# johnmatthewtennant/wab-gym

Measured on AMD Instinct MI355X. Metric: env-steps/sec (whole node) at batch=65536; obs bit-exact vs CPU ref, higher is better.
Workload: dtype u8

## Files before the change

wab_gym_amd/csrc/wab_build_guard.h:

```cpp
#pragma once

#if defined(WAB_STAMPS) || defined(WAB2_STAMPS) || defined(WAB_ROLL_FLOOR) || defined(WAB_WIDE_ROLL_FLOOR) || \
    defined(WAB2_ABLATE) || defined(WAB_ONLY_WAVE)
#if defined(WAB_PRODUCT_BUILD)
#error "a diagnostic macro (WAB_STAMPS, WAB2_STAMPS, WAB_ROLL_FLOOR, WAB_WIDE_ROLL_FLOOR, WAB2_ABLATE, WAB_ONLY_WAVE) is set in the product build"
#elif !defined(WAB_DIAGNOSTIC_BUILD)
#error "diagnostic macros need -DWAB_DIAGNOSTIC_BUILD and an output outside the product library (tools/build_variants.sh)"
#endif
#endif

#ifndef WAB_RULES_INSTANCE
#define WAB_RULES_INSTANCE 1
#endif
#ifndef WAB_ROLL_HOIST
#define WAB_ROLL_HOIST 1
#endif
#if defined(WAB_PRODUCT_BUILD) && (WAB_RULES_INSTANCE != 1 || WAB_ROLL_HOIST != 1)
#error "WAB_RULES_INSTANCE / WAB_ROLL_HOIST are A/B switches: the product build takes their defaults"
#endif

#if defined(WAB_DIAGNOSTIC_BUILD) && !defined(__HIP_DEVICE_COMPILE__)
extern "C" __attribute__((weak, visibility("default"))) int wab_diagnostic_build(void) { return 1; }
#endif
```

wab_gym_amd/csrc/wab_step_small.hip:

```cpp
#include <hip/hip_runtime.h>

#include "wab_default_rules.h"
#include "wab_feat.h"
#include "wab_policy_dev.h"

#ifndef WAB_ROLL_THROTTLE
#define WAB_ROLL_THROTTLE 0
#endif
#ifndef WAB_ROLL_OBS_NT
#define WAB_ROLL_OBS_NT 1
#endif
namespace wab {

#ifdef WAB_STAMPS
#define SMALL_STAMP(slot)                                                                \
  do {                                                                                   \
    if (lane == 0 && p.stamps && (!ROLL || t == p.n_steps / 2))                          \
      p.stamps[(size_t)blockIdx.x * kStampStride + (slot)] = __builtin_amdgcn_s_memrealtime();      \
  } while (0)
#else
#define SMALL_STAMP(slot) do {} while (0)
#endif

namespace {
// ... 249 lines not shown
constexpr int kW1ResetPrio = 2;

template <bool ROLL>
__device__ __forceinline__ void role_prio(uint32_t level, int t, bool rot) {
  if (ROLL && rot)
    set_prio_dyn((level >= 2u ? 1u : 0u) + 2u * (((blockIdx.x >> 8) + (uint32_t)t) & 1u));
  else
    set_prio_dyn(level);
}
constexpr int kStripW1 = 8;
__device__ __forceinline__ M128 strip_of(const Params& p, const Lds& s, int lane, int dir) {
  return strip_cells(p, dir, s.strip[lane] | s.strip[64 + lane]);
}

__device__ __forceinline__ void scan_log(const Params& p, const Head& h, const uint32_t* lxy, const uint32_t* lrem,
                                         int i0, int ne, int& found, int& found_rem, M128& gone) {
#pragma unroll
  for (int k = 0; k < 4; ++k) {
    const bool in = i0 + k < ne;
    const uint32_t v = lxy[k];
    const int r = (int)lrem[k];
    if (in && v == h.cpos) {
      found = i0 + k;
      found_rem = r;
    }
    const int ddx = h.ox - xy_x(v), ddy = h.oy - xy_y(v);
    set_bit_if(gone, (uint32_t)((ddx + p.cw) * p.H + ddy + p.ch), in && r == 0 && abs(ddx) <= p.cw && abs(ddy) <= p.ch);
  }
}

__device__ __forceinline__ void stream_set_ostrich(const Params& p, uint32_t* stream, uint32_t ebit, int role) {
  const uint32_t ccb = (uint32_t)(p.cw * p.H + p.ch);
  if (p.restrict_view && m_test(view_mask_of(p, role), ccb)) return;
  const uint32_t bit = ebit + 2u * (uint32_t)p.WH + ccb;
  atomicOr(&stream[bit >> 5], 1u << (bit & 31u));
}

__device__ __forceinline__ void render_s(const Params& p, const Lds& s, int lane, uint32_t info, int dir) {
  const uint32_t WH = (uint32_t)p.WH;
  const uint32_t ebit = (uint32_t)lane * (uint32_t)p.OB;
  const int role = (int)((info >> 8) & 0xFFu);
  M128 wp = m_unpack(s.wolfp[lane]);
  M128 bp = m_or(m_unpack(s.bushp[lane]), m_andn(strip_of(p, s, lane, dir), m_unpack(s.gone[lane])));
  if (p.restrict_view) {
    const M128 vm = view_mask_of(p, role);
    wp = m_andn(wp, vm);
    bp = m_andn(bp, vm);
  }
  if (wp.lo | wp.hi) stream_or128(s.stream, ebit, wp);
  stream_or128(s.stream, ebit + WH, bp);
  stream_set_ostrich(p, s.stream, ebit, role);
}


#ifndef WAB_STORE_WHOLE
#define WAB_STORE_WHOLE 1
#endif
constexpr uint32_t kUnits11 = 64u * 363u / 16u;
template <int NT, int K0, int K1, int I0>
__device__ __forceinline__ void store_units_whole11(uint8_t* out, uint32_t* stream, int lane) {
  typedef uint32_t u32x4 __attribute__((ext_vector_type(4)));
  typedef u32x4 __attribute__((may_alias)) u32x4_any;
  static_assert(I0 % 64 == 0 && NT % 64 == 0, "a wave's units of one k are contiguous");
  static_assert((uint32_t)(I0 + NT * K0) < kUnits11, "the wave has a unit");
  const uint16_t* s16 = reinterpret_cast<const uint16_t*>(stream) + I0;
  uint32_t v[K1 - K0];
  uint32_t share_end = 0u;
#pragma unroll
  for (int k = K0; k < K1; ++k) {
    const uint32_t u0 = (uint32_t)(I0 + NT * k);
    if (u0 + 63u < kUnits11) v[k - K0] = (uint32_t)s16[lane + NT * k];
    else if (u0 < kUnits11) v[k - K0] = (uint32_t)s16[min((uint32_t)lane, kUnits11 - 1u - u0) + NT * k];
    else v[k - K0] = 0u;
    if (u0 < kUnits11) share_end = min((u0 + 64u) * 2u, (kUnits11 * 2u + 15u) & ~15u);
  }
#pragma unroll
  for (int i = 0; i < (K1 - K0 + 7) / 8; ++i) {
    const uint32_t k = (uint32_t)(K0 + 8 * i) + ((uint32_t)lane >> 3);
    const uint32_t byte = ((uint32_t)I0 + (uint32_t)NT * k) * 2u + 16u * ((uint32_t)lane & 7u);
    *reinterpret_cast<u32x4_any*>(reinterpret_cast<uint8_t*>(stream) + min(byte, share_end - 16u)) = u32x4{0u, 0u, 0u, 0u};
  }
  if (!out) return;
  typedef uint8_t __attribute__((address_space(1))) g_u8;
  typedef u32x4 __attribute__((address_space(1))) g_u32x4;
  g_u8* base = (g_u8*)out;
  uint32_t base_off = 0u;
#pragma unroll
  for (int k = K0; k < K1; ++k) {
    const uint32_t u0 = (uint32_t)(I0 + NT * k);
    if (u0 >= kUnits11) continue;
    const uint32_t adv = ((uint32_t)(NT * k) * 16u - base_off) & ~4095u;
    if (adv) {
      base += adv;
      base_off += adv;
      asm("" : "+s"(base));
    }
    if (u0 + 63u >= kUnits11 && u0 + (uint32_t)lane >= kUnits11) continue;
    u32x4 q;
#pragma unroll
    for (int b = 0; b < 4; ++b) q[b] = (((v[k - K0] >> (4 * b)) & 0xFu) * 0x00204081u) & 0x01010101u;
    g_u32x4* dst = (g_u32x4*)base + (uint32_t)(I0 + lane + NT * k - (int)(base_off / 16u));
    if (WAB_ROLL_OBS_NT) __builtin_nontemporal_store(q, dst);
    else *dst = q;
  }
}

template <int G, int NT, int NK, int I0>
__device__ __forceinline__ void store_units_nt(const Params& p, uint8_t* planes, uint32_t* stream, int lane) {
  const int64_t g0 = (int64_t)blockIdx.x * 64;
  const uint32_t OB = (uint32_t)p.OB;
  if (WAB_STORE_WHOLE && G == 11 && p.B - g0 >= 64) {
    store_units_whole11<NT, 0, NK, I0>(planes ? planes + (size_t)g0 * OB : nullptr, stream, lane);
    return;
  }
  const int idx = I0 + lane;
  const uint32_t full = ((uint32_t)min((int64_t)64, p.B - g0) * OB) >> 4;
  uint8_t* out = planes + (size_t)g0 * OB;
  uint16_t* s16 = reinterpret_cast<uint16_t*>(stream);
  uint32_t v[NK];
#pragma unroll
  for (int k = 0; k < NK; ++k) {
    const uint32_t u = (uint32_t)(idx + NT * k);
    v[k] = u < full ? (uint32_t)s16[u] : 0u;
  }
#pragma unroll
  for (int k = 0; k < NK; ++k) {
    const uint32_t u = (uint32_t)(idx + NT * k);
    if (u < full) s16[u] = 0;
  }
  if (!planes) return;
#pragma unroll
  for (int k = 0; k < NK; ++k) {
    const uint32_t u = (uint32_t)(idx + NT * k);
    if (u >= full) continue;
    typedef uint32_t u32x4 __attribute__((ext_vector_type(4)));
    u32x4 q;
#pragma unroll
    for (int b = 0; b < 4; ++b) q[b] = (((v[k] >> (4 * b)) & 0xFu) * 0x00204081u) & 0x01010101u;
    if (WAB_ROLL_OBS_NT) __builtin_nontemporal_store(q, reinterpret_cast<u32x4*>(out) + u);
    else reinterpret_cast<u32x4*>(out)[u] = q;
  }
}

#ifndef WAB_ROLL_FLOOR
#define WAB_ROLL_FLOOR 0
#endif

struct CarryHdr {
  uint4 hdr;
};
struct CarryW0 {
  uint8_t* prev_planes;
  uint32_t* prev_stream;
  uint4 hdr;
  double food;
  uint32_t bw[4];
  uint32_t lxy[4], lrem[4];
};
template <int SLOTS>
struct CarryW2 {
  static constexpr int NR = carry_reg_slots(SLOTS);
  uint8_t* prev_planes;
  uint32_t* prev_stream;
  uint4 hdr;
  uint32_t wr[NR > 0 ? NR : 1];
  uint32_t live;
};

template <typename C>
struct CarryPtr {
  uint8_t* prev_planes;
  uint32_t* prev_stream;
  C c;
};

__device__ __forceinline__ int act_of(const Lds& s, int lane) {
  return (int)reinterpret_cast<const int8_t*>(s.act)[lane];
}

__device__ __forceinline__ void prefetch_actions(const Params& p, const Lds& s, int lane) {
  const int64_t g0 = (int64_t)blockIdx.x * 64;
  const int8_t* a = p.actions + p.B + g0;
  if (g0 + 64 <= p.B && (reinterpret_cast<uintptr_t>(a) & 3u) == 0u) {
    typedef const uint32_t __attribute__((address_space(4))) CU32;
    CU32* c = (CU32*)reinterpret_cast<uintptr_t>(a);
    asm volatile("" : "+s"(c));
    uint32_t v[16];
#pragma unroll
    for (int k = 0; k < 16; ++k) v[k] = c[k];
    uint32_t d = 0;
#pragma unroll
    for (int k = 0; k < 16; ++k) d = lane == k ? v[k] : d;
    if (lane < 16) s.act[lane] = d;
  } else {
    const int8_t v = g0 + lane < p.B ? a[lane] : (int8_t)0;
    reinterpret_cast<int8_t*>(s.act)[lane] = v;
  }
}

// ... 132 lines not shown
    bw0 = carry->bw[0];
    bw1 = carry->bw[1];
    bw2 = carry->bw[2];
    bw3 = carry->bw[3];
#pragma unroll
    for (int i = 0; i < 4; ++i) {
      lxy[i] = carry->lxy[i];
      lrem[i] = carry->lrem[i];
    }
  } else {
  hr = head_fetch<COLD>(p, g, active);
  {
    const int64_t gl = active ? g : 0;
    food = cold_of<COLD>(p).food[gl];
    bw0 = cold_of<COLD>(p).bushmap[gl];
    if (p.WHW > 1) bw1 = cold_of<COLD>(p).bushmap[p.B + gl];
    if (p.WHW > 2) bw2 = cold_of<COLD>(p).bushmap[2 * p.B + gl];
    if (p.WHW > 3) bw3 = cold_of<COLD>(p).bushmap[3 * p.B + gl];
#pragma unroll
    for (int i = 0; i < 4; ++i) {
      const int64_t at = (int64_t)min(i, p.eaten_cap - 1) * p.B + gl;
      lxy[i] = cold_of<COLD>(p).eaten_xy[at];
      lrem[i] = cold_of<COLD>(p).eaten_rem[at];
    }
  }
  opaque_head(hr);
  opaque(food);
  opaque(bw0);
  opaque(bw1);
  opaque(bw2);
  opaque(bw3);
#pragma unroll
  for (int i = 0; i < 4; ++i) {
    opaque(lxy[i]);
    opaque(lrem[i]);
  }
  }
  if (!active) {
    food = 0.0;
    bw0 = bw1 = bw2 = bw3 = 0u;
  }
  const bool init = !ROLL || t == 0;
  if (init) {
    uint4* z = reinterpret_cast<uint4*>(s.stream);
    for (uint32_t i = lane; i < L.stream_words / 4u; i += 64) z[i] = make_uint4(0u, 0u, 0u, 0u);
  }
  if (ROLL && pol) hr.a = act_of(s, lane);
  const Head h = head_decode(p, g, active, hr);
  if (lane == 0 && init) {
    s.flag[0] = 0u;
    s.flag[1] = 0u;
  }
  if (init) lds_barrier();
  int ne = (int)misc_ne(h.hdr.z), ndep = (int)misc_ndep(h.hdr.z);
  if (ROLL && t == 0) {
    for (int i = 4; i < kSmallLog; ++i)
      if (active && i < ne && i < p.eaten_cap) {
        s.elxy[(i - 4) * 64 + lane] = cold_of<COLD>(p).eaten_xy[(int64_t)i * p.B + g];
        s.elrem[(i - 4) * 64 + lane] = cold_of<COLD>(p).eaten_rem[(int64_t)i * p.B + g];
      }
    __builtin_amdgcn_s_waitcnt(0);
  }
  const int status_old = (int)misc_status(h.hdr.z);
  const int role = h.role;
  M128 bm = m_make(bw0, bw1, bw2, bw3);
  if (h.dir == DIR_RIGHT || h.dir == DIR_UP) shl128(bm.lo, bm.hi, h.dir == DIR_RIGHT ? p.H : 1);
  else if (h.dir == DIR_LEFT || h.dir == DIR_DOWN) shr128(bm.lo, bm.hi, h.dir == DIR_LEFT ? p.H : 1);
  {
    const M128 valid = m_make(sreg(p.small_masks[2][0]), sreg(p.small_masks[2][1]), sreg(p.small_masks[2][2]),
                              sreg(p.small_masks[2][3]));
    const M128 col0 = m_make(sreg(p.small_masks[0][0]), sreg(p.small_masks[0][1]), sreg(p.small_masks[0][2]),
                             sreg(p.small_masks[0][3]));
    const M128 coll = m_make(sreg(p.small_masks[1][0]), sreg(p.small_masks[1][1]), sreg(p.small_masks[1][2]),
                             sreg(p.small_masks[1][3]));
    const bool up = h.dir == DIR_UP, down = h.dir == DIR_DOWN;
    const M128 drop = {sel64(up, col0.lo, 0ull) | sel64(down, coll.lo, 0ull),
                       sel64(up, col0.hi, 0ull) | sel64(down, coll.hi, 0ull)};
    bm = m_andn(m_and(bm, valid), drop);
  }
  SMALL_STAMP(1);
  SMALL_STAMP(2);
  int found = -1, found_rem = 0;
  M128 gone = {0ull, 0ull};
  scan_log(p, h, lxy, lrem, 0, ne, found, found_rem, gone);
  bm = m_andn(bm, gone);
  bool center_bush = m_test(bm, ccb);
  if (ne > 4 && (center_bush || (ndep > 0 && h.dir != DIR_STAY))) {
    const int i_hbm = ROLL ? kSmallLog : 4;
    if (ROLL)
      for (int i0 = 4; i0 < ne && i0 < kSmallLog; i0 += 4) {
        uint32_t exy[4], erem[4];
#pragma unroll
        for (int k = 0; k < 4; ++k) {
          exy[k] = s.elxy[(i0 + k - 4) * 64 + lane];
          erem[k] = s.elrem[(i0 + k - 4) * 64 + lane];
        }
        scan_log(p, h, exy, erem, i0, ne, found, found_rem, gone);
      }
    for (int i0 = i_hbm; i0 < ne; i0 += 4) {
      uint32_t exy[4] = {0u, 0u, 0u, 0u}, erem[4] = {0u, 0u, 0u, 0u};
#pragma unroll
      for (int k = 0; k < 4; ++k)
        if (i0 + k < ne) {
          exy[k] = cold_of<COLD>(p).eaten_xy[(int64_t)(i0 + k) * p.B + g];
          erem[k] = cold_of<COLD>(p).eaten_rem[(int64_t)(i0 + k) * p.B + g];
        }
      scan_log(p, h, exy, erem, i0, ne, found, found_rem, gone);
    }
    bm = m_andn(bm, gone);
    center_bush = m_test(bm, ccb);
  }
  SMALL_STAMP(7);
  s.bushp[lane] = m_pack(bm);
  s.gone[lane] = m_pack(gone);
  int rem = found_rem;
  if (found < 0) {
    rem = 0;
    if (center_bush) {
      lds_await(p, s.flag);
      rem = (int)s.cval[lane];
    }
  }
  SMALL_STAMP(8);
  double reward = 0.0;
  unsigned long long eaten_of = 0;
  const bool ate = rem > 0 && status_old == 0 && (role == 1 || p.lookout_only);
  if (ate) {
    food = food + p.fill;
    food = food < 0.0 ? 0.0 : (food > 1.0 ? 1.0 : food);
    reward += p.r_eat;
    bool logged = true;
    if (ROLL && found >= 0 && found < 4) {
#pragma unroll
      for (int k = 0; k < 4; ++k)
        if (found == k) lrem[k] = (uint32_t)(rem - 1);
    } else if (ROLL && found < 0 && ne < 4 && ne < p.eaten_cap) {
#pragma unroll
      for (int k = 0; k < 4; ++k)
        if (ne == k) {
          lxy[k] = h.cpos;
          lrem[k] = (uint32_t)(rem - 1);
        }
      ne += 1;
    } else if (ROLL && found >= 4 && found < kSmallLog) {
      s.elrem[(found - 4) * 64 + lane] = (uint8_t)(rem - 1);
    } else if (ROLL && found < 0 && ne >= 4 && ne < kSmallLog && ne < p.eaten_cap) {
      s.elxy[(ne - 4) * 64 + lane] = h.cpos;
      s.elrem[(ne - 4) * 64 + lane] = (uint8_t)(rem - 1);
      ne += 1;
    } else if (found >= 0) {
      cold_of<COLD>(p).eaten_rem[(int64_t)found * p.B + g] = (uint8_t)(rem - 1);
    } else if (ne < p.eaten_cap) {
      cold_of<COLD>(p).eaten_xy[(int64_t)ne * p.B + g] = h.cpos;
      cold_of<COLD>(p).eaten_rem[(int64_t)ne * p.B + g] = (uint8_t)(rem - 1);
      ne += 1;
    } else {
      eaten_of += 1;
      logged = false;
    }
    if (rem == 1) {
      m_clear(bm, ccb);
      if (logged) ndep += 1;
    }
  }
  food = food - p.hunger;
  const bool starved = food <= 0.0;
  if (starved) food = 0.0;
  s.info[lane] = (starved ? 1u : 0u) | ((uint32_t)role << 8) | ((uint32_t)ne << 16) | ((uint32_t)ndep << 24);
  SMALL_STAMP(3);
  lds_barrier();
  role_prio<ROLL>(1, t, p.features != nullptr);

  const bool killed = s.kill[lane] != 0u;
  const int status = starved ? 1 : killed ? 2 : status_old;
  const bool done = env_done(p, h, starved, killed);
  {
    const double r_finish = sreg(p.r_finish), r_turn = sreg(p.r_turn);
    const double r_starve = sreg(p.r_starve), r_killed = sreg(p.r_killed);
    reward += sel_f64(status == 0, sel_f64(done, r_finish, r_turn), sel_f64(status == 1, r_starve, r_killed));
  }
  const bool job = active && done && p.autoreset;
  if (ROLL && p.returns)
    s.rcode[64 * t + lane] = reward_code(ate, status, done);
  if (active) {
    const int ft = (int)ceil(food * (double)p.turns_empty);
    __builtin_nontemporal_store((float)reward, p.reward + g);
    __builtin_nontemporal_store((uint8_t)(done ? 1 : 0), p.done + g);
    uint8_t* fts = reinterpret_cast<uint8_t*>(sel64(job, (uint64_t)p.t_food_turns, (uint64_t)p.food_turns));
    uint8_t* rls = reinterpret_cast<uint8_t*>(sel64(job, (uint64_t)p.t_role, (uint64_t)p.role));
    uint8_t* sts = reinterpret_cast<uint8_t*>(sel64(job, (uint64_t)p.t_status, (uint64_t)p.status));
    if (!job || (!ROLL && p.t_planes)) {
      fts[g] = (uint8_t)ft;
      rls[g] = (uint8_t)role;
      sts[g] = (uint8_t)status;
    }
    if (p.features && !job) s.scal[lane] = (uint32_t)ft | ((uint32_t)role << 8) | ((uint32_t)status << 16);
    if (!job) {
      bm = m_or(bm, m_andn(strip_of(p, s, lane, h.dir), gone));
      if (!ROLL || last) {
        cold_of<COLD>(p).bushmap[g] = m_word<0>(bm);
        if (p.WHW > 1) cold_of<COLD>(p).bushmap[p.B + g] = m_word<1>(bm);
        if (p.WHW > 2) cold_of<COLD>(p).bushmap[2 * p.B + g] = m_word<2>(bm);
        if (p.WHW > 3) cold_of<COLD>(p).bushmap[3 * p.B + g] = m_word<3>(bm);
        cold_of<COLD>(p).food[g] = food;
      }
    }
  }
  if (eaten_of) atomicAdd(&cold_of<COLD>(p).counters[CTR_EATEN_OVERFLOW], eaten_of);
  if (active && !h.valid_action) atomicAdd(&cold_of<COLD>(p).counters[CTR_BAD_ACTIONS], 1ull);
  if (blockIdx.x == 0 && threadIdx.x == 0)
    atomicAdd(&cold_of<COLD>(p).counters[CTR_STEPS], (unsigned long long)p.B);
  const unsigned long long jm = __ballot(job);
  if (lane == 0 && jm) atomicAdd(&p.block_resets[blockIdx.x], (unsigned long long)__popcll(jm));
  if (ROLL && carry->prev_stream) store_units_nt<G, 128, 12, 0>(p, carry->prev_planes, carry->prev_stream, lane);
  SMALL_STAMP(4);
  lds_barrier();
  if (!ROLL && p.t_planes) {
    unsigned long long wolf_of = 0;
    if (jm) {
      uint8_t* tout = p.t_planes + (size_t)g0 * OB;
      for (unsigned long long jj = jm; jj; jj &= jj - 1) {
        const uint32_t ee = (uint32_t)(__ffsll(jj) - 1);
        for (uint32_t k = lane; k < OB; k += 64) {
          const uint32_t bit = ee * OB + k;
          tout[bit] = (uint8_t)((s.stream[bit >> 5] >> (bit & 31)) & 1u);
        }
      }
      asm volatile("s_waitcnt lgkmcnt(0)" ::: "memory");
      if (job) {
        const uint32_t ebit = (uint32_t)lane * OB;
        stream_clear(s.stream, ebit, OB);
        const int j = __popcll(jm & ((1ull << lane) - 1ull));
        const uint2 kq = *reinterpret_cast<const uint2*>(&s.jkey[2 * j]);
        const int role2 = new_episode_a<SLOTS>(p, s, h, g, kq.x, kq.y, ebit, wolf_of);
        new_episode_b(p, s, g, j, ebit, role2);
      }
    }
    if (wolf_of) atomicAdd(&cold_of<COLD>(p).counters[CTR_WOLF_OVERFLOW], wolf_of);
    lds_barrier();
  }
  if constexpr (ROLL) {
    if (!last) {
      if (job) {
        const NewEp n = carry_of(s, lane);
        const int j = __popcll(jm & ((1ull << lane) - 1ull));
        const uint4 nb = *reinterpret_cast<const uint4*>(&s.jbm[4 * j]);
        carry->hdr = new_header(n, h);
        carry->food = n.food;
        carry->bw[0] = nb.x;
        carry->bw[1] = nb.y;
        carry->bw[2] = nb.z;
// ... 12 lines not shown
        carry->lxy[i] = lxy[i];
        carry->lrem[i] = lrem[i];
      }
    } else if (active && !job) {
#pragma unroll
      for (int i = 0; i < 4; ++i)
        if (i < ne && i < p.eaten_cap) {
          cold_of<COLD>(p).eaten_xy[(int64_t)i * p.B + g] = lxy[i];
          cold_of<COLD>(p).eaten_rem[(int64_t)i * p.B + g] = (uint8_t)lrem[i];
        }
      for (int i = 4; i < kSmallLog; ++i)
        if (i < ne && i < p.eaten_cap) {
          cold_of<COLD>(p).eaten_xy[(int64_t)i * p.B + g] = s.elxy[(i - 4) * 64 + lane];
          cold_of<COLD>(p).eaten_rem[(int64_t)i * p.B + g] = s.elrem[(i - 4) * 64 + lane];
        }
    }
  }
  if (ROLL && last && p.returns) rollout_returns<COLD>(p, s, g, active, lane);
  SMALL_STAMP(5);
  return jm;
}

template <int G, bool ROLL = false, bool COLD = false>
__device__ __forceinline__ unsigned long long draws_wave(const Params& p, const SmallLayout& L, uint32_t* lds, int lane,
                                                         CarryHdr* carry = nullptr, int t = 0, bool last = true,
                                                         bool pol = false) {
  const Lds s = lds_of(lds, L);
  const int64_t g = (int64_t)blockIdx.x * 64 + lane;
  SMALL_STAMP(10);
  role_prio<ROLL>(2, t, p.features != nullptr);
  HeadRaw hr;
  if (ROLL && t > 0) {
    hr.hdr = carry->hdr;
    hr.a = act_of(s, lane);
  } else {
  hr = head_fetch<COLD>(p, g, g < p.B);
  {
    const int nthr = p.max_berries;
    uint64_t tv[4];
#pragma unroll
    for (int k = 0; k < 4; ++k) tv[k] = cold_of<COLD>(p).thresholds[min(64 * k + lane, max(nthr, 1) - 1)];
    opaque_head(hr);
#pragma unroll
    for (int k = 0; k < 4; ++k) opaque(tv[k]);
#pragma unroll
    for (int k = 0; k < 4; ++k)
      if (64 * k + lane < nthr) s.thr[64 * k + lane] = tv[k];
    if (lane == 0) bush_thr_pads(s.thr, nthr);
  }
  }
  if (ROLL && pol) hr.a = act_of(s, lane);
  const Head h = head_decode(p, g, g < p.B, hr);
  if (!ROLL || t == 0) lds_barrier();
  SMALL_STAMP(30);
  const uint64_t ek = mix64(h.kenv ^ (uint64_t)h.hdr.w);
  const uint32_t b0 = (uint32_t)ek, b1 = (uint32_t)(ek >> 32);
  SMALL_STAMP(31);
  s.cval[lane] =
      (uint32_t)bush_value_fast(s.thr, p.max_berries, draw_U(h.cpos, make_ts(SITE_BUSH, 0, 0), b0, b1), p.bush_power);
  lds_publish(s.flag);
  role_prio<ROLL>(0, t, p.features != nullptr);
  if (p.features && !p.restrict_view && !ROLL)
    early_view_zeros(p, 0u, (uint32_t)min((int64_t)32, p.B - (int64_t)blockIdx.x * 64), lane);
  SMALL_STAMP(11);
  s.strip[lane] = strip_draws(p, h, b0, b1, 0, kStripW1);
  SMALL_STAMP(12);
  lds_barrier();
  const uint32_t info = s.info[lane];
  const bool killed = s.kill[lane] != 0u;
  const bool job = h.active && p.autoreset && env_done(p, h, info_starved(info), killed);
  const unsigned long long jm = __ballot(job);
  if (jm) {
    if (ROLL) role_prio<ROLL>(kW1ResetPrio, t, p.features != nullptr);
    if (job) {
      const uint64_t ek2 = mix64(h.kenv ^ (uint64_t)(h.hdr.w + 1u));
      const int j = __popcll(jm & ((1ull << lane) - 1ull));
      *reinterpret_cast<uint2*>(&s.jkey[2 * j]) = make_uint2((uint32_t)ek2, (uint32_t)(ek2 >> 32));
    }
    reset_chunk(p, s.tiles, s.jkey, __popcll(jm), 0u, lane, s.jbm);
    lds_publish(&s.flag[1]);
    if (ROLL) role_prio<ROLL>(0, t, p.features != nullptr);
  }
  if (h.active && (!job || (!ROLL && p.t_planes))) {
    render_s(p, s, lane, info, h.dir);
  }
  if (ROLL && !last && !pol) prefetch_actions(p, s, lane);
  SMALL_STAMP(13);
  lds_barrier();
  if (!ROLL && p.t_planes) lds_barrier();
  SMALL_STAMP(14);
  if (ROLL && lane == 0) {
    s.flag[0] = 0u;
    s.flag[1] = 0u;
  }
  if (ROLL && !last) {
    const uint32_t status = info_starved(info) ? 1u : killed ? 2u : misc_status(h.hdr.z);
    carry->hdr = job ? new_header(carry_of(s, lane), h)
                     : make_uint4(h.cpos, (uint32_t)h.turn, misc_pack((uint32_t)h.role, status, 0u, 0u, 0u), h.hdr.w);
  }
  return jm;
}

template <int SLOTS, int G, bool ROLL = false, bool COLD = false>
__device__ __forceinline__ unsigned long long wolves_wave(const Params& p, const SmallLayout& L, uint32_t* lds, int lane,
                                                          CarryW2<SLOTS>* carry = nullptr, int t = 0, bool last = true,
                                                          bool pol = false) {
  const Lds s = lds_of(lds, L);
  const int64_t g = (int64_t)blockIdx.x * 64 + lane;
  const bool active = g < p.B;
  SMALL_STAMP(16);
#ifndef WAB_SPEC_WOLVES
#define WAB_SPEC_WOLVES 8
#endif
  constexpr int kSpecSlots = SLOTS < WAB_SPEC_WOLVES ? SLOTS : WAB_SPEC_WOLVES;
  uint32_t wr[SLOTS];
#pragma unroll
  for (int k = 0; k < SLOTS; ++k) wr[k] = 0u;
  HeadRaw hr;
  const bool carried = ROLL && t > 0;
  if (carried) {
    hr.hdr = carry->hdr;
    hr.a = act_of(s, lane);
    constexpr int NR = CarryW2<SLOTS>::NR;
#pragma unroll
    for (int k = 0; k < SLOTS; ++k) wr[k] = k < NR ? carry->wr[k < NR ? k : 0] : s.wcar[(k - NR) * 64 + lane];
  } else {
  {
    const int64_t gl = active ? g : 0;
#pragma unroll
    for (int k = 0; k < kSpecSlots; ++k) wr[k] = cold_of<COLD>(p).wolves[(int64_t)k * p.B + gl];
  }
  hr = head_fetch<COLD>(p, g, active);
  opaque_head(hr);
#pragma unroll
  for (int k = 0; k < kSpecSlots; ++k) opaque(wr[k]);
  }
  if (ROLL && pol) hr.a = act_of(s, lane);
  const Head h = head_decode(p, g, active, hr);
  if (!ROLL || t == 0) lds_barrier();
  SMALL_STAMP(28);
  const int nw = (int)misc_nw(h.hdr.z);
  if (!carried) {
#pragma unroll
    for (int k = kSpecSlots; k < SLOTS; ++k)
      if (k < nw) wr[k] = cold_of<COLD>(p).wolves[(int64_t)k * p.B + g];
  }
  const uint64_t ek = mix64(h.kenv ^ (uint64_t)h.hdr.w);
  const uint32_t b0 = (uint32_t)ek, b1 = (uint32_t)(ek >> 32);
  uint32_t live = carried ? (h.active ? carry->live : 0u) : nw >= 32 ? ~0u : ((1u << nw) - 1u);

  {
    uint32_t keep = 0;
#pragma unroll
    for (int g4 = 0; g4 < SLOTS; g4 += 4) {
      const uint32_t live4 = (live >> g4) & 0xFu;
      if (!live4) continue;
      uint32_t h1[4], hh[4], ts[4];
#pragma unroll
      for (int q = 0; q < 4; ++q) {
        const int k = g4 + q;
        uint32_t occ = 0;
#pragma unroll
        for (int t = 0; t < k; ++t) occ += (((live >> t) & 1u) && wr[t] == wr[k]) ? 1u : 0u;
        ts[q] = make_ts(SITE_DESPAWN, occ, h.turn);
        h1[q] = wr[k] ^ b0;
      }
      fmix32x4(h1);
#pragma unroll
      for (int q = 0; q < 4; ++q) hh[q] = h1[q] ^ ts[q] ^ b1;
      fmix32x4(hh);
      uint32_t kp = 0, tie = 0;
#pragma unroll
      for (int q = 0; q < 4; ++q) {
        kp |= (hh[q] > p.keep_th ? 1u : 0u) << q;
        tie |= (hh[q] == p.keep_th ? 1u : 0u) << q;
      }
      if (tie & live4) {
#pragma unroll
        for (int q = 0; q < 4; ++q)
          if (((tie >> q) & 1u) && draw_lo21(h1[q], ts[q], b0) >= p.keep_tl) kp |= 1u << q;
      }
      keep |= (kp & live4) << g4;
    }
    live = keep;
  }
  SMALL_STAMP(29);
  M128 wolfp = {0ull, 0ull};
  bool kill = false;
#pragma unroll
  for (int g4 = 0; g4 < SLOTS; g4 += 4) {
    if (!((live >> g4) & 0xFu)) continue;
#pragma unroll
    for (int q = 0; q < 4; ++q) {
      const int k = g4 + q;
      const bool on = (live >> k) & 1u;
      int wx = xy_x(wr[k]), wy = xy_y(wr[k]);
      if (p.wolves_can_move) {
        const int ddx = h.ox - wx, ddy = h.oy - wy;
        const bool alongx = abs(ddx) >= abs(ddy);
        wx += alongx ? sgn(ddx) : 0;
        wy += alongx ? 0 : sgn(ddy);
        wr[k] = xy_pack(wx, wy);
      }
      const int ddx = h.ox - wx, ddy = h.oy - wy;
      set_bit_if(wolfp, (uint32_t)((ddx + p.cw) * p.H + ddy + p.ch), on && abs(ddx) <= p.cw && abs(ddy) <= p.ch);
      kill |= on && ddx == 0 && ddy == 0;
    }
  }
  kill = kill && !p.god_mode;
  s.wolfp[lane] = m_pack(wolfp);
  s.kill[lane] = kill ? 1u : 0u;
  SMALL_STAMP(17);
  SMALL_STAMP(18);
  lds_barrier();
  const uint32_t info = s.info[lane];
  const bool starved = info_starved(info);
  const bool job = active && p.autoreset && env_done(p, h, starved, kill);

  unsigned long long wolf_of = 0;
  const M128 spawn = m_unpack(s.spawn[lane]);
  if (active && (spawn.lo | spawn.hi)) {
#pragma unroll
    for (int half = 0; half < 2; ++half) {
      uint64_t bits = half ? spawn.hi : spawn.lo;
      while (bits) {
        const int b = __ffsll((unsigned long long)bits) - 1;
        bits &= bits - 1;
        const int r = 64 * half + b;
        const uint32_t w = xy_add(h.cpos, G == 11 ? ring11(r) : cold_of<COLD>(p).tables[p.ring_at + r]);
        bool placed = false;
#pragma unroll
        for (int k = 0; k < SLOTS; ++k)
          if (!placed && !((live >> k) & 1u)) { wr[k] = w; live |= 1u << k; placed = true; }
        if (!placed) wolf_of += 1;
      }
    }
  }
  if (active && !job && (!ROLL || last)) {
    int n = 0;
#pragma unroll
    for (int k = 0; k < SLOTS; ++k)
      if ((live >> k) & 1u) cold_of<COLD>(p).wolves[(int64_t)(n++) * p.B + g] = wr[k];
    const uint32_t status = starved ? 1u : kill ? 2u : misc_status(h.hdr.z);
    cold_of<COLD>(p).hdr[g] = make_uint4(h.cpos, (uint32_t)h.turn,
                          misc_pack((info >> 8) & 0xFFu, status, (uint32_t)n, (info >> 16) & 0xFFu, info >> 24),
                          h.hdr.w);
  }
  if (wolf_of) atomicAdd(&cold_of<COLD>(p).counters[CTR_WOLF_OVERFLOW], wolf_of);
  const unsigned long long jm = __ballot(job);
  if (ROLL && carry->prev_stream) store_units_nt<G, 128, 12, 64>(p, carry->prev_planes, carry->prev_stream, lane);
  SMALL_STAMP(19);
  lds_barrier();
  if (!ROLL && p.t_planes) lds_barrier();
  SMALL_STAMP(20);
  if (ROLL && !last) {
    if (job) {
      const NewEp n = carry_of(s, lane);
      M128 m = n.wolves;
      constexpr int NR = CarryW2<SLOTS>::NR;
#pragma unroll
      for (int k = 0; k < SLOTS; ++k) {
        const bool any = (m.lo | m.hi) != 0ull;
        const uint32_t c = m.lo ? (uint32_t)(__ffsll((unsigned long long)m.lo) - 1)
                                : (uint32_t)(__ffsll((unsigned long long)m.hi) + 63);
        const uint32_t w = any ? s.tiles[any ? c : 0u] : 0u;
        if (k < NR) carry->wr[k < NR ? k : 0] = w;
        else s.wcar[(k - NR) * 64 + lane] = w;
        if (any) m_clear(m, c);
      }
      carry->live = n.nw >= 32u ? ~0u : ((1u << n.nw) - 1u);
// ... 13 lines not shown
                              h.hdr.w);
    }
  }
  return jm;
}

template <int SLOTS, int G, bool ROLL = false, bool COLD = false>
__device__ __forceinline__ unsigned long long ring_wave(const Params& p, const SmallLayout& L, uint32_t* lds, int lane,
                                                        CarryHdr* carry = nullptr, int t = 0, bool last = true,
                                                        bool pol = false) {
  const Lds s = lds_of(lds, L);
  const int64_t g = (int64_t)blockIdx.x * 64 + lane;
  SMALL_STAMP(22);
  if (ROLL) role_prio<ROLL>(0, t, p.features != nullptr);
  HeadRaw hr;
  if (ROLL && t > 0) {
    hr.hdr = carry->hdr;
    hr.a = act_of(s, lane);
    reinterpret_cast<uint4*>(s.jbm)[lane] = make_uint4(0u, 0u, 0u, 0u);
  } else {
  hr = head_fetch<COLD>(p, g, g < p.B);
  if constexpr (G == 11) {
    for (int c = lane; c < 121; c += 64) s.tiles[c] = xy_pack(5 - c / 11, 5 - c % 11);
  } else {
    uint32_t tv[2];
#pragma unroll
    for (int k = 0; k < 2; ++k) tv[k] = cold_of<COLD>(p).tables[min(64 * k + lane, p.WH - 1)];
#pragma unroll
    for (int k = 0; k < 2; ++k)
      if (64 * k + lane < p.WH) s.tiles[64 * k + lane] = tv[k];
  }
  reinterpret_cast<uint4*>(s.jbm)[lane] = make_uint4(0u, 0u, 0u, 0u);
  {
    const int n = p.n_gap + 1;
    uint64_t gv[3];
#pragma unroll
    for (int k = 0; k < 3; ++k) gv[k] = cold_of<COLD>(p).gap[min(64 * k + lane, n - 1)];
    opaque_head(hr);
#pragma unroll
    for (int k = 0; k < 3; ++k) opaque(gv[k]);
#pragma unroll
    for (int k = 0; k < 3; ++k)
      if (64 * k + lane < n) s.gap[64 * k + lane] = gv[k];
  }
  }
  if (p.features) {
    uint4* z = reinterpret_cast<uint4*>(lds + L.fbits);
    const uint32_t nz = ROLL && t > 0 ? L.ftab - L.fbits : L.fzero;
    for (uint32_t i = lane; i < nz / 4u; i += 64) z[i] = make_uint4(0u, 0u, 0u, 0u);
  }
  if (ROLL && pol) hr.a = act_of(s, lane);
  const Head h = head_decode(p, g, g < p.B, hr);
  if (!ROLL || t == 0) lds_barrier();
  if (p.features) {
    if (!ROLL || t == 0)
      feat_tables_build(feat_tables_at(lds + L.ftab, p.W / 2 + p.H / 2 + 1), p.W, p.H, p.W / 2 + p.H / 2 + 1, lane, 64);
    if (!p.restrict_view && !ROLL)
      early_view_zeros(p, 32u, (uint32_t)max((int64_t)0, min((int64_t)32, p.B - (int64_t)blockIdx.x * 64 - 32)), lane);
  }
  const uint64_t ek = mix64(h.kenv ^ (uint64_t)h.hdr.w);
  const uint32_t b0 = (uint32_t)ek, b1 = (uint32_t)(ek >> 32);
  M128 spawn = {0ull, 0ull};
  if (p.wolves_on && h.active)
    spawn_hits(s.gap, p.R, p.gap_full_th, p.gap_full_tl, p.gap_ring_th, p.gap_ring_tl, p.gap_inv_l2, h.turn, b0, b1, [&](int r) { m_set(spawn, (uint32_t)r); });
  s.spawn[lane] = m_pack(spawn);
  s.strip[64 + lane] = strip_draws(p, h, b0, b1, kStripW1, 1 << 30);
  SMALL_STAMP(23);
  lds_barrier();
  role_prio<ROLL>(3, t, p.features != nullptr);
  const bool job = h.active && p.autoreset && env_done(p, h, info_starved(s.info[lane]), s.kill[lane] != 0u);
  const unsigned long long jm = __ballot(job);
  int role2 = 0;
  if (jm) {
    const int j = __popcll(jm & ((1ull << lane) - 1ull));
    uint32_t* jkey = s.jkey + 2 * 64;
    uint64_t ek2 = 0;
    if (job) {
      ek2 = mix64(h.kenv ^ (uint64_t)(h.hdr.w + 1u));
      *reinterpret_cast<uint2*>(&jkey[2 * j]) = make_uint2((uint32_t)ek2, (uint32_t)(ek2 >> 32));
    }
    const int n_jobs = __popcll(jm);
    for (uint32_t c0 = 64; c0 < (uint32_t)p.WH; c0 += 64)
      reset_chunk(p, s.tiles, jkey, n_jobs, c0, lane, s.jbm);
    SMALL_STAMP(24);
    if (ROLL || !p.t_planes) {
      unsigned long long wolf_of = 0;
      const uint32_t ebit = (uint32_t)lane * (uint32_t)p.OB;
      if (job) role2 = new_episode_a<SLOTS, ROLL, COLD>(p, s, h, g, (uint32_t)ek2, (uint32_t)(ek2 >> 32), ebit, wolf_of, last);
      lds_await(p, &s.flag[1]);
      SMALL_STAMP(9);
      if (job) new_episode_b<COLD>(p, s, g, j, ebit, role2, !ROLL || last);
      if (wolf_of) atomicAdd(&cold_of<COLD>(p).counters[CTR_WOLF_OVERFLOW], wolf_of);
    }
  }
  SMALL_STAMP(25);
  lds_barrier();
  if (!ROLL && p.t_planes) lds_barrier();
  SMALL_STAMP(26);
  if (ROLL && !last) {
    const uint32_t status = info_starved(s.info[lane]) ? 1u : s.kill[lane] != 0u ? 2u : misc_status(h.hdr.z);
    carry->hdr = job ? new_header(carry_of(s, lane), h)
                     : make_uint4(h.cpos, (uint32_t)h.turn, misc_pack((uint32_t)h.role, status, 0u, 0u, 0u), h.hdr.w);
  }
  return jm;
}

template <int G, int K0, int K1, int WAVE>
__device__ __forceinline__ void store_units_of(const Params& p, uint32_t* stream, int lane) {
  const int64_t g0 = (int64_t)blockIdx.x * 64;
  const uint32_t OB = (uint32_t)p.OB;
  if (WAB_STORE_WHOLE && G == 11 && p.B - g0 >= 64) {
    store_units_whole11<256, K0, K1, 64 * WAVE>(p.planes + (size_t)g0 * OB, stream, lane);
    return;
  }
  const int tid = 64 * WAVE + lane;
  const uint32_t full = ((uint32_t)min((int64_t)64, p.B - g0) * OB) >> 4;
  uint8_t* out = p.planes + (size_t)g0 * OB;
  uint16_t* s16 = reinterpret_cast<uint16_t*>(stream);
  uint32_t v[K1 - K0];
#pragma unroll
  for (int k = K0; k < K1; ++k) {
    const uint32_t u = (uint32_t)tid + 256u * (uint32_t)k;
    v[k - K0] = u < full ? (uint32_t)s16[u] : 0u;
  }
#pragma unroll
  for (int k = K0; k < K1; ++k) {
    const uint32_t u = (uint32_t)tid + 256u * (uint32_t)k;
    if (u < full) s16[u] = 0;
  }
#pragma unroll
  for (int k = K0; k < K1; ++k) {
    const uint32_t u = (uint32_t)tid + 256u * (uint32_t)k;
    if (u >= full) break;
    typedef uint32_t u32x4 __attribute__((ext_vector_type(4)));
    u32x4 q;
#pragma unroll
    for (int b = 0; b < 4; ++b) q[b] = (((v[k - K0] >> (4 * b)) & 0xFu) * 0x00204081u) & 0x01010101u;
    if (WAB_ROLL_OBS_NT) __builtin_nontemporal_store(q, reinterpret_cast<u32x4*>(out) + u);
    else reinterpret_cast<u32x4*>(out)[u] = q;
  }
}

template <bool CLEAR = false>
__device__ __forceinline__ void store_obs(const Params& p, uint32_t* stream, int tid) {
  const int64_t g0 = (int64_t)blockIdx.x * 64;
  const uint32_t OB = (uint32_t)p.OB;
  const uint32_t limit = (uint32_t)min((int64_t)64, p.B - g0) * OB;
  uint8_t* out = p.planes + (size_t)g0 * OB;
  const uint16_t* s16 = reinterpret_cast<const uint16_t*>(stream);
  const uint32_t full = limit >> 4;
  uint32_t v[6];
#pragma unroll
  for (int k = 0; k < 6; ++k) {
    const uint32_t u = (uint32_t)tid + 256u * (uint32_t)k;
    v[k] = u < full ? (uint32_t)s16[u] : 0u;
  }
  if constexpr (CLEAR) {
    uint16_t* w16 = reinterpret_cast<uint16_t*>(stream);
#pragma unroll
    for (int k = 0; k < 6; ++k) {
      const uint32_t u = (uint32_t)tid + 256u * (uint32_t)k;
      if (u < full) w16[u] = 0;
    }
  }
#pragma unroll
  for (int k = 0; k < 6; ++k) {
    const uint32_t u = (uint32_t)tid + 256u * (uint32_t)k;
    if (u >= full) break;
    typedef uint32_t u32x4 __attribute__((ext_vector_type(4)));
    u32x4 q;
#pragma unroll
    for (int b = 0; b < 4; ++b) q[b] = (((v[k] >> (4 * b)) & 0xFu) * 0x00204081u) & 0x01010101u;
#ifndef WAB_STEP_OBS_NT
#define WAB_STEP_OBS_NT 1
#endif
    if (WAB_STEP_OBS_NT) __builtin_nontemporal_store(q, reinterpret_cast<u32x4*>(out) + u);
    else reinterpret_cast<u32x4*>(out)[u] = q;
  }
  for (uint32_t b = (full << 4) + tid; b < limit; b += 256)
    out[b] = (uint8_t)((stream[b >> 5] >> (b & 31)) & 1u);
#ifdef WAB_STAMPS
  asm volatile("s_waitcnt vmcnt(0)" ::: "memory");
  if ((tid & 63) == 0 && p.stamps) {
    const int slot[4] = {6, 15, 21, 27};
    p.stamps[(size_t)blockIdx.x * kStampStride + slot[tid >> 6]] = __builtin_amdgcn_s_memrealtime();
  }
#endif
}

template <bool ROLL = false, bool POLICY = false>
__device__ __forceinline__ void step_features(const Params& p, const SmallLayout& L, uint32_t* lds, int wave,
                                              int lane, int t = 0, float* rows = nullptr) {
  const int md = p.W / 2 + p.H / 2 + 1;
  const uint32_t F = (uint32_t)pragmatic_dim(md, p.turns_empty), WH = (uint32_t)p.WH;
  const int64_t g0 = (int64_t)blockIdx.x * 64;
  const uint32_t n_active = (uint32_t)min((int64_t)64, p.B - g0);
  const uint32_t* stream = lds + L.stream;
  uint32_t* ob = lds + L.fbits;
  if (ROLL && (uint32_t)lane < n_active) {
    const uint32_t ebit = (uint32_t)lane * (uint32_t)p.OB, at = (uint32_t)lane * F;
    const FeatTables ft = feat_tables_at(lds + L.ftab, md);
    if (wave <= 1) {
      uint32_t near, second;
      plane_nearest(ft, md, stream_get128(stream, ebit + (uint32_t)wave * WH, WH), near, second);
      emit_nearest(ob, at, wave, md, near, second);
    } else if (wave == 2) {
#pragma unroll
      for (int pl = 0; pl < 2; ++pl) {
        int counts[4];
        plane_counts(ft, stream_get128(stream, ebit + (uint32_t)pl * WH, WH), counts);
        emit_counts(ob, at, pl, md, counts);
      }
    } else {
      const uint32_t sc = lds[L.scal + lane];
      const uint32_t role = (sc >> 8) & 0xFFu;
      const uint32_t sb_bit = ebit + WH + (uint32_t)(md / 2) * (uint32_t)p.S + (uint32_t)(md / 2);
      emit_scalars(ob, at, md, p.turns_empty, (stream[sb_bit >> 5] >> (sb_bit & 31u)) & 1u, sc & 0xFFu, role,
                   sc >> 16, p.restrict_view != 0, view_mask_of(p, (int)role));
    }
  } else if ((uint32_t)lane < n_active && wave < 3) {
    const uint32_t ebit = (uint32_t)lane * (uint32_t)p.OB, at = (uint32_t)lane * F;
    if (wave <= 1) {
      uint32_t near, second;
      int counts[4];
      plane_features(feat_tables_at(lds + L.ftab, md), md, stream_get128(stream, ebit + (uint32_t)wave * WH, WH), near,
                     second, counts);
      emit_plane(ob, at, wave, md, near, second, counts);
    } else {
      const uint32_t sc = lds[L.scal + lane];
      const uint32_t role = (sc >> 8) & 0xFFu;
      const uint32_t sb_bit = ebit + WH + (uint32_t)(md / 2) * (uint32_t)p.S + (uint32_t)(md / 2);
      emit_scalars(ob, at, md, p.turns_empty, (stream[sb_bit >> 5] >> (sb_bit & 31u)) & 1u, sc & 0xFFu, role,
                   sc >> 16, p.restrict_view != 0, view_mask_of(p, (int)role));
    }
  }
#ifdef WAB_STAMPS
  const auto stamp = [&](int slot) {
    if (ROLL && threadIdx.x == 0 && p.stamps && t == p.n_steps / 2)
      p.stamps[(size_t)blockIdx.x * kStampStride + slot] = __builtin_amdgcn_s_memrealtime();
  };
// ... 187 lines not shown
  p.block_resets = r.block_resets; p.n_steps = r.n_steps;
  p.t_planes = nullptr; p.t_food_turns = r.food_turns; p.t_role = r.role; p.t_status = r.status;
}

template <int SLOTS, int G, bool FEAT, bool ROLL, bool RULES, bool POLICY>
__global__ __launch_bounds__(256) __attribute__((amdgpu_waves_per_eu(POLICY ? 2 : ROLL ? 4 : 1))) void wab_step_small(Params p0) {
  static_assert(!POLICY || (FEAT && ROLL), "the policy build is a build of wab_rollout_features' kernel");
  extern __shared__ __attribute__((aligned(16))) uint32_t lds[];
#ifdef WAB_STAMPS
  uint64_t t_entry;
  asm volatile("s_memrealtime %0\n\ts_waitcnt lgkmcnt(0)" : "=s"(t_entry)::"memory");
#endif
  if ((int64_t)blockIdx.x * 64 >= p0.B) return;
#ifdef WAB_STAMPS
  if (threadIdx.x == 0 && p0.stamps) {
    uint32_t xcc;
    asm volatile("s_getreg_b32 %0, hwreg(HW_REG_XCC_ID)" : "=s"(xcc));
    p0.stamps[(size_t)blockIdx.x * kStampStride + 34] = __builtin_amdgcn_s_memrealtime();
    p0.stamps[(size_t)blockIdx.x * kStampStride + 32] = t_entry;
    p0.stamps[(size_t)blockIdx.x * kStampStride + 33] = xcc & 0xFu;
  }
#endif
  const int wave = __builtin_amdgcn_readfirstlane(threadIdx.x >> 6), lane = threadIdx.x & 63;
#ifdef WAB_STAMPS
  if (lane == 0 && p0.stamps) {
    uint32_t hw;
    asm volatile("s_getreg_b32 %0, hwreg(HW_REG_HW_ID)" : "=s"(hw));
    p0.stamps[(size_t)blockIdx.x * kStampStride + 40 + wave] = hw;
  }
#endif
#ifdef WAB_ONLY_WAVE
  if (wave != WAB_ONLY_WAVE) return;
#endif
  if constexpr (!ROLL) {
    unsigned long long jm;
    if (wave == 0) {
      __builtin_amdgcn_s_setprio(3);
      const Params p = wave_params<G, FEAT, RULES>(p0);
      jm = bushes_wave<SLOTS, G>(p, small_layout(p), lds, lane);
      __builtin_amdgcn_s_setprio(0);
    } else if (wave == 1) {
      const Params p = wave_params<G, FEAT, RULES>(p0);
      jm = draws_wave<G>(p, small_layout(p), lds, lane);
    } else if (wave == 2) {
      const Params p = wave_params<G, FEAT, RULES>(p0);
      jm = wolves_wave<SLOTS, G>(p, small_layout(p), lds, lane);
    } else {
      const Params p = wave_params<G, FEAT, RULES>(p0);
      jm = ring_wave<SLOTS, G>(p, small_layout(p), lds, lane);
    }
    const Params p = wave_params<G, FEAT, RULES>(p0);
    const SmallLayout L = small_layout(p);
    (void)jm;
    if (!FEAT || p.planes) store_obs(p, lds + L.stream, threadIdx.x);
    if constexpr (FEAT) step_features(p, L, lds, wave, lane);
  } else {
    const int T = p0.n_steps;
    constexpr bool HOIST = WAB_ROLL_HOIST && RULES && !FEAT;
#ifdef WAB_STAMPS
#define ROLL_LOOP_STAMP(slot, cond)                                                          \
  do {                                                                                       \
    if (threadIdx.x == 0 && p0.stamps && (cond))                                             \
      p0.stamps[(size_t)blockIdx.x * kStampStride + (slot)] = __builtin_amdgcn_s_memrealtime();         \
  } while (0)
#else
#define ROLL_LOOP_STAMP(slot, cond) do {} while (0)
#endif
    {
      const SmallLayout L = small_layout(wave_params<G, FEAT, RULES>(p0));
      uint4* z = reinterpret_cast<uint4*>(lds + L.stream2);
      for (uint32_t i = threadIdx.x; i < L.stream_words / 4u; i += 256) z[i] = make_uint4(0u, 0u, 0u, 0u);
    }
#define WAB_ROLL_STEP(...)                                                                   \
    RollSlices io = roll_slices(wave_params<G, FEAT, RULES>(p0));                            \
    if constexpr (POLICY) {   \
      const Params p = wave_params<G, FEAT, RULES>(p0);                                      \
      const int64_t g = (int64_t)blockIdx.x * 64 + lane;                                     \
      const uint4 h0 = p.hdr[g < p.B ? g : 0];                                               \
      roll_policy<true>(p, small_layout(p), lds, wave, lane, h0.w, h0.y, 0);                 \
      lds_barrier();                                                                         \
    }                                                                                        \
    for (int t = 0; t < T; ++t) {                                                            \
      ROLL_LOOP_STAMP(35, t == T / 2);   \
      if (WAB_ROLL_THROTTLE && (wave == 0 || wave == 2)) __builtin_amdgcn_s_waitcnt(0x0F70);  \
      Params p = wave_params<G, FEAT, RULES>(p0);                                            \
      if constexpr (HOIST) {                                                                 \
        if (t > 0) roll_advance(io);                                                         \
        roll_apply(p, io);                                                                   \
      } else {                                                                               \
        step_slice(p, t);                                                                    \
      }                                                                                      \
      float* rows = nullptr;      \
      if constexpr (POLICY) {                                                                \
        p.features = p.pol.features_last;              \
        rows = t == T - 1 ? p.pol.features_last                                              \
               : p.pol.features ? p.pol.features + (int64_t)(t + 1) * p.B * p.pol.d.F : nullptr; \
      }                                                                                      \
      const SmallLayout L0 = small_layout(p);                                                \
      SmallLayout L = L0;                                                                    \
      if (t & 1) L.stream = L0.stream2;                                                      \
      c.prev_planes = !p.planes ? nullptr : HOIST ? p.planes - io.d_planes : p.planes - (int64_t)p.B * p.OB; \
      c.prev_stream = t > 0 ? lds + ((t & 1) ? L0.stream : L0.stream2) : nullptr;           \
      if (WAB_ROLL_FLOOR) {   \
        lds_barrier();                                                                       \
        if constexpr (kWave == 0 || kWave == 2) {          \
          if (c.prev_stream) store_units_nt<G, 128, 12, 32 * kWave>(p, c.prev_planes, c.prev_stream, lane); \
        }                                                                                    \
// ... 89 lines not shown
```

Before: 14.42 billion.

## Split step-path rendering into bush/wolf waves and use whole-unit obs store

In the non-rolled step kernel, each wave now renders its own part of the observation (the bush wave ORs bushes and the strip into the stream, the wolf wave ORs wolves) directly from registers. This replaces staging bushp, gone and wolfp in LDS and a later render_s pass. For G==11 full blocks, store_obs now uses the per-wave store_units_whole11 path without clearing the stream instead of the generic loop. A diagnostic WAB_STEP_FLOOR early-exit is also added. The cost is concurrent stream_or128 writes from different waves, whose ordering relies on the existing barriers.

```diff
diff --git a/wab_gym_amd/csrc/wab_build_guard.h b/wab_gym_amd/csrc/wab_build_guard.h
--- a/wab_gym_amd/csrc/wab_build_guard.h
+++ b/wab_gym_amd/csrc/wab_build_guard.h
@@ -1,9 +1,9 @@
 #pragma once
 
 #if defined(WAB_STAMPS) || defined(WAB2_STAMPS) || defined(WAB_ROLL_FLOOR) || defined(WAB_WIDE_ROLL_FLOOR) || \
-    defined(WAB2_ABLATE) || defined(WAB_ONLY_WAVE)
+    defined(WAB_STEP_FLOOR) || defined(WAB2_ABLATE) || defined(WAB_ONLY_WAVE)
 #if defined(WAB_PRODUCT_BUILD)
-#error "a diagnostic macro (WAB_STAMPS, WAB2_STAMPS, WAB_ROLL_FLOOR, WAB_WIDE_ROLL_FLOOR, WAB2_ABLATE, WAB_ONLY_WAVE) is set in the product build"
+#error "a diagnostic macro (WAB_STAMPS, WAB2_STAMPS, WAB_ROLL_FLOOR, WAB_WIDE_ROLL_FLOOR, WAB_STEP_FLOOR, WAB2_ABLATE, WAB_ONLY_WAVE) is set in the product build"
 #elif !defined(WAB_DIAGNOSTIC_BUILD)
 #error "diagnostic macros need -DWAB_DIAGNOSTIC_BUILD and an output outside the product library (tools/build_variants.sh)"
 #endif
@@ -15,8 +15,15 @@
 #ifndef WAB_ROLL_HOIST
 #define WAB_ROLL_HOIST 1
 #endif
-#if defined(WAB_PRODUCT_BUILD) && (WAB_RULES_INSTANCE != 1 || WAB_ROLL_HOIST != 1)
-#error "WAB_RULES_INSTANCE / WAB_ROLL_HOIST are A/B switches: the product build takes their defaults"
+#ifndef WAB_STEP_RENDER_SPLIT
+#define WAB_STEP_RENDER_SPLIT 1
+#endif
+#ifndef WAB_STEP_STORE_WHOLE
+#define WAB_STEP_STORE_WHOLE 1
+#endif
+#if defined(WAB_PRODUCT_BUILD) && \
+    (WAB_RULES_INSTANCE != 1 || WAB_ROLL_HOIST != 1 || WAB_STEP_RENDER_SPLIT != 1 || WAB_STEP_STORE_WHOLE != 1)
+#error "WAB_RULES_INSTANCE / WAB_ROLL_HOIST / WAB_STEP_RENDER_SPLIT / WAB_STEP_STORE_WHOLE are A/B switches: the product build takes their defaults"
 #endif
 
 #if defined(WAB_DIAGNOSTIC_BUILD) && !defined(__HIP_DEVICE_COMPILE__)
diff --git a/wab_gym_amd/csrc/wab_step_small.hip b/wab_gym_amd/csrc/wab_step_small.hip
--- a/wab_gym_amd/csrc/wab_step_small.hip
+++ b/wab_gym_amd/csrc/wab_step_small.hip
@@ -325,12 +325,25 @@
   stream_set_ostrich(p, s.stream, ebit, role);
 }
 
+[[maybe_unused]] __device__ __forceinline__ void render_wolves(const Params& p, const Lds& s, int lane, uint32_t info, M128 wp) {
+  if (p.restrict_view) wp = m_andn(wp, view_mask_of(p, (int)((info >> 8) & 0xFFu)));
+  if (wp.lo | wp.hi) stream_or128(s.stream, (uint32_t)lane * (uint32_t)p.OB, wp);
+}
+[[maybe_unused]] __device__ __forceinline__ void render_bushes(const Params& p, const Lds& s, int lane, int role, const M128& bush,
+                                              const M128& strip) {
+  const uint32_t ebit = (uint32_t)lane * (uint32_t)p.OB;
+  M128 bp = m_or(bush, strip);
+  if (p.restrict_view) bp = m_andn(bp, view_mask_of(p, role));
+  stream_or128(s.stream, ebit + (uint32_t)p.WH, bp);
+  stream_set_ostrich(p, s.stream, ebit, role);
+}
+
 
 #ifndef WAB_STORE_WHOLE
 #define WAB_STORE_WHOLE 1
 #endif
 constexpr uint32_t kUnits11 = 64u * 363u / 16u;
-template <int NT, int K0, int K1, int I0>
+template <int NT, int K0, int K1, int I0, bool CLEAR = true>
 __device__ __forceinline__ void store_units_whole11(uint8_t* out, uint32_t* stream, int lane) {
   typedef uint32_t u32x4 __attribute__((ext_vector_type(4)));
   typedef u32x4 __attribute__((may_alias)) u32x4_any;
@@ -348,7 +361,7 @@
     if (u0 < kUnits11) share_end = min((u0 + 64u) * 2u, (kUnits11 * 2u + 15u) & ~15u);
   }
 #pragma unroll
-  for (int i = 0; i < (K1 - K0 + 7) / 8; ++i) {
+  for (int i = 0; CLEAR && i < (K1 - K0 + 7) / 8; ++i) {
     const uint32_t k = (uint32_t)(K0 + 8 * i) + ((uint32_t)lane >> 3);
     const uint32_t byte = ((uint32_t)I0 + (uint32_t)NT * k) * 2u + 16u * ((uint32_t)lane & 7u);
     *reinterpret_cast<u32x4_any*>(reinterpret_cast<uint8_t*>(stream) + min(byte, share_end - 16u)) = u32x4{0u, 0u, 0u, 0u};
@@ -418,6 +431,19 @@
 #ifndef WAB_ROLL_FLOOR
 #define WAB_ROLL_FLOOR 0
 #endif
+#ifndef WAB_STEP_FLOOR
+#define WAB_STEP_FLOOR 0
+#endif
+template <bool ROLL>
+constexpr bool kRenderSplit = WAB_STEP_RENDER_SPLIT && !ROLL;
+template <bool ROLL>
+constexpr bool kStepFloor = WAB_STEP_FLOOR && !ROLL;
+[[maybe_unused]] __device__ __forceinline__ unsigned long long step_floor_tail(const Params& p) {
+  lds_barrier();
+  lds_barrier();
+  if (p.t_planes) lds_barrier();
+  return 0ull;
+}
 
 struct CarryHdr {
   uint4 hdr;
@@ -656,6 +682,7 @@
     s.flag[1] = 0u;
   }
   if (init) lds_barrier();
+  if constexpr (kStepFloor<ROLL>) return step_floor_tail(p);
   int ne = (int)misc_ne(h.hdr.z), ndep = (int)misc_ndep(h.hdr.z);
   if (ROLL && t == 0) {
     for (int i = 4; i < kSmallLog; ++i)
@@ -715,8 +742,11 @@
     center_bush = m_test(bm, ccb);
   }
   SMALL_STAMP(7);
-  s.bushp[lane] = m_pack(bm);
-  s.gone[lane] = m_pack(gone);
+  const M128 bush_s = bm;
+  if constexpr (!kRenderSplit<ROLL>) {
+    s.bushp[lane] = m_pack(bush_s);
+    s.gone[lane] = m_pack(gone);
+  }
   int rem = found_rem;
   if (found < 0) {
     rem = 0;
@@ -784,6 +814,15 @@
     reward += sel_f64(status == 0, sel_f64(done, r_finish, r_turn), sel_f64(status == 1, r_starve, r_killed));
   }
   const bool job = active && done && p.autoreset;
+  M128 strip = {0ull, 0ull};
+  if constexpr (kRenderSplit<ROLL>) {
+    SMALL_STAMP(44);
+    if (active && (!job || p.t_planes)) {
+      strip = m_andn(strip_of(p, s, lane, h.dir), gone);
+      render_bushes(p, s, lane, role, bush_s, strip);
+    }
+    SMALL_STAMP(45);
+  }
   if (ROLL && p.returns)
     s.rcode[64 * t + lane] = reward_code(ate, status, done);
   if (active) {
@@ -800,7 +839,8 @@
     }
     if (p.features && !job) s.scal[lane] = (uint32_t)ft | ((uint32_t)role << 8) | ((uint32_t)status << 16);
     if (!job) {
-      bm = m_or(bm, m_andn(strip_of(p, s, lane, h.dir), gone));
+      if constexpr (!kRenderSplit<ROLL>) strip = m_andn(strip_of(p, s, lane, h.dir), gone);
+      bm = m_or(bm, strip);
       if (!ROLL || last) {
         cold_of<COLD>(p).bushmap[g] = m_word<0>(bm);
         if (p.WHW > 1) cold_of<COLD>(p).bushmap[p.B + g] = m_word<1>(bm);
@@ -919,6 +959,7 @@
   if (ROLL && pol) hr.a = act_of(s, lane);
   const Head h = head_decode(p, g, g < p.B, hr);
   if (!ROLL || t == 0) lds_barrier();
+  if constexpr (kStepFloor<ROLL>) return step_floor_tail(p);
   SMALL_STAMP(30);
   const uint64_t ek = mix64(h.kenv ^ (uint64_t)h.hdr.w);
   const uint32_t b0 = (uint32_t)ek, b1 = (uint32_t)(ek >> 32);
@@ -948,8 +989,10 @@
     lds_publish(&s.flag[1]);
     if (ROLL) role_prio<ROLL>(0, t, p.features != nullptr);
   }
-  if (h.active && (!job || (!ROLL && p.t_planes))) {
-    render_s(p, s, lane, info, h.dir);
+  if constexpr (!kRenderSplit<ROLL>) {
+    if (h.active && (!job || (!ROLL && p.t_planes))) {
+      render_s(p, s, lane, info, h.dir);
+    }
   }
   if (ROLL && !last && !pol) prefetch_actions(p, s, lane);
   SMALL_STAMP(13);
@@ -1005,6 +1048,7 @@
   if (ROLL && pol) hr.a = act_of(s, lane);
   const Head h = head_decode(p, g, active, hr);
   if (!ROLL || t == 0) lds_barrier();
+  if constexpr (kStepFloor<ROLL>) return step_floor_tail(p);
   SMALL_STAMP(28);
   const int nw = (int)misc_nw(h.hdr.z);
   if (!carried) {
@@ -1075,7 +1119,7 @@
     }
   }
   kill = kill && !p.god_mode;
-  s.wolfp[lane] = m_pack(wolfp);
+  if constexpr (!kRenderSplit<ROLL>) s.wolfp[lane] = m_pack(wolfp);
   s.kill[lane] = kill ? 1u : 0u;
   SMALL_STAMP(17);
   SMALL_STAMP(18);
@@ -1083,6 +1127,11 @@
   const uint32_t info = s.info[lane];
   const bool starved = info_starved(info);
   const bool job = active && p.autoreset && env_done(p, h, starved, kill);
+  if constexpr (kRenderSplit<ROLL>) {
+    SMALL_STAMP(46);
+    if (active && (!job || p.t_planes)) render_wolves(p, s, lane, info, wolfp);
+    SMALL_STAMP(47);
+  }
 
   unsigned long long wolf_of = 0;
   const M128 spawn = m_unpack(s.spawn[lane]);
@@ -1202,6 +1251,7 @@
   if (ROLL && pol) hr.a = act_of(s, lane);
   const Head h = head_decode(p, g, g < p.B, hr);
   if (!ROLL || t == 0) lds_barrier();
+  if constexpr (kStepFloor<ROLL>) return step_floor_tail(p);
   if (p.features) {
     if (!ROLL || t == 0)
       feat_tables_build(feat_tables_at(lds + L.ftab, p.W / 2 + p.H / 2 + 1), p.W, p.H, p.W / 2 + p.H / 2 + 1, lane, 64);
@@ -1291,10 +1341,32 @@
   }
 }
 
-template <bool CLEAR = false>
+__device__ __forceinline__ void store_obs_stamp(const Params& p, int tid) {
+#ifdef WAB_STAMPS
+  asm volatile("s_waitcnt vmcnt(0)" ::: "memory");
+  if ((tid & 63) == 0 && p.stamps) {
+    const int slot[4] = {6, 15, 21, 27};
+    p.stamps[(size_t)blockIdx.x * kStampStride + slot[tid >> 6]] = __builtin_amdgcn_s_memrealtime();
+  }
+#endif
+}
+
+template <int G, bool CLEAR = false>
 __device__ __forceinline__ void store_obs(const Params& p, uint32_t* stream, int tid) {
   const int64_t g0 = (int64_t)blockIdx.x * 64;
   const uint32_t OB = (uint32_t)p.OB;
+  if constexpr (WAB_STEP_STORE_WHOLE && G == 11 && !CLEAR) {
+    if (p.B - g0 >= 64) {
+      const int wave = __builtin_amdgcn_readfirstlane(tid >> 6), lane = tid & 63;
+      uint8_t* out = p.planes + (size_t)g0 * OB;
+      if (wave == 0) store_units_whole11<256, 0, 6, 0, false>(out, stream, lane);
+      else if (wave == 1) store_units_whole11<256, 0, 6, 64, false>(out, stream, lane);
+      else if (wave == 2) store_units_whole11<256, 0, 6, 128, false>(out, stream, lane);
+      else store_units_whole11<256, 0, 6, 192, false>(out, stream, lane);
+      store_obs_stamp(p, tid);
+      return;
+    }
+  }
   const uint32_t limit = (uint32_t)min((int64_t)64, p.B - g0) * OB;
   uint8_t* out = p.planes + (size_t)g0 * OB;
   const uint16_t* s16 = reinterpret_cast<const uint16_t*>(stream);
@@ -1329,13 +1401,7 @@
   }
   for (uint32_t b = (full << 4) + tid; b < limit; b += 256)
     out[b] = (uint8_t)((stream[b >> 5] >> (b & 31)) & 1u);
-#ifdef WAB_STAMPS
-  asm volatile("s_waitcnt vmcnt(0)" ::: "memory");
-  if ((tid & 63) == 0 && p.stamps) {
-    const int slot[4] = {6, 15, 21, 27};
-    p.stamps[(size_t)blockIdx.x * kStampStride + slot[tid >> 6]] = __builtin_amdgcn_s_memrealtime();
-  }
-#endif
+  store_obs_stamp(p, tid);
 }
 
 template <bool ROLL = false, bool POLICY = false>
@@ -1629,7 +1695,7 @@
     const Params p = wave_params<G, FEAT, RULES>(p0);
     const SmallLayout L = small_layout(p);
     (void)jm;
-    if (!FEAT || p.planes) store_obs(p, lds + L.stream, threadIdx.x);
+    if (!FEAT || p.planes) store_obs<G>(p, lds + L.stream, threadIdx.x);
     if constexpr (FEAT) step_features(p, L, lds, wave, lane);
   } else {
     const int T = p0.n_steps;
```

New measurement: 14.45 billion (median of 3 runs). About the same (+0.2%).
